# rmqtt/rmqtt

Measured on NVIDIA H100. Metric: topic-matches/sec @10M subs, higher is better.
Workload: dtype u32

## Files before the change

rmqtt_b200/csrc/engine.cu:

```cuda
#include <cuda_runtime.h>
#include <sched.h>
#include <sys/syscall.h>
#include <unistd.h>

#include <algorithm>
#include <cctype>
#include <cstddef>
#include <cstdio>
#include <cstdlib>
#include <cstring>
#include <condition_variable>
#include <mutex>
#include <string>
#include <type_traits>
#include <vector>

#include "../../include/gpumqtt.h"
#include "host_trie.h"
#include "comm.cuh"
#include "pipeline.cuh"
#include "relations.cuh"
#include "retain_tree.h"
#include "router_host.h"

// ... 320 lines not shown
            if (stage_used_) { CUDA_TRY(cudaEventRecord(ev_arena_[arena_], side)); arena_pending_[arena_] = true; }
            dev_view = trie_view(trie, d_edges.as<EdgeSlot>(), d_ranges.as<Range>(), d_values.as<u32>(), d_dict.as<DictSlot>(), d_pool.as<u8>(), d_cfilter.as<u32>(),
                                 d_tree_slots.as<u32>());
            dev_rview = retain_view(rtree, d_rkids.as<RKid>(), d_redges.as<REdge>(), d_rvals.as<u32>());
            view_epoch++;
            CUDA_TRY(cudaEventRecord(ev_flush, side));
            flush_gen++;
        }
        if (r_shipped) rtree.shipped();
        return GM_OK;
    }

    std::vector<MatchCtx*> all_ctxs() { std::vector<MatchCtx*> v; for (auto& c : ctxs) v.push_back(&c); v.push_back(&devctx); return v; }

    struct MatchCall : MatchIO {
        u64* d_needed = nullptr;
        bool keep_cursor = false;
        bool timing = true;
        u32 site_bits = 0;
    };
    int enqueue_match(MatchCtx& c, MatchCall a, cudaStream_t s) {
        if (a.n == 0) { if (a.d_needed) CUDA_TRY(cudaMemsetAsync(a.d_needed, 0, sizeof(u64), s)); return GM_OK; }
        if (a.n > 0xFFFFFFF0ull) { g_err = "batch too large"; return GM_ERR_TOO_LARGE; }
        if (a.cap > 0xFFFFFFFFull) a.cap = 0xFFFFFFFFull;
        MatchKnobs kn = knobs;
        if (a.site_bits) { kn.site_bits = a.site_bits; kn.sub_bits = 0; }
        const bool small = a.hdr != nullptr;
        const MatchPlan p = plan_match(static_cast<u32>(a.n), dev_view.max_depth, kn, num_sms, small);
        CUDA_TRY(c.d_tok.ensure(p.tok));
        CUDA_TRY(c.d_tok8.ensure(p.tok8));
        CUDA_TRY(c.d_meta.ensure(p.meta));
        CUDA_TRY(c.d_slow.ensure(p.slow));
        CUDA_TRY(c.d_ctrl.ensure(p.ctrl));
        CUDA_TRY(c.d_sort.ensure(p.sort));
        CUDA_TRY(c.d_hist.ensure(p.hist));
        CUDA_TRY(c.d_gstack.ensure(p.gstack));
        CUDA_TRY(c.d_gpool.ensure(p.gpool));
        if (!small) {
            CUDA_TRY(cudaStreamWaitEvent(s, ev_flush, 0));
            if (c.recorded) CUDA_TRY(cudaStreamWaitEvent(s, c.ev_done, 0));
        }
        if (a.keep_cursor) CUDA_TRY(cudaMemsetAsync(static_cast<char*>(c.d_ctrl.p) + sizeof(unsigned long long), 0, sizeof(Ctrl) - sizeof(unsigned long long), s));
        else CUDA_TRY(cudaMemsetAsync(c.d_ctrl.p, 0, sizeof(Ctrl), s));
        CUDA_TRY(cudaMemsetAsync(c.d_hist.p, 0, p.nbuckets * sizeof(u32), s));
        MatchScratch m{};
        m.tok = c.d_tok.as<u32>(); m.tok8 = c.d_tok8.as<u32>(); m.meta = c.d_meta.as<u32>(); m.slow = c.d_slow.as<u32>(); m.sort = c.d_sort.as<u32>(); m.hist = c.d_hist.as<u32>();
        m.ctrl = c.d_ctrl.as<Ctrl>(); m.gstack = c.d_gstack.as<u64>(); m.gpool = c.d_gpool.as<Desc>();
        cudaEvent_t* ev_t = ev_ring[ring_n % RING];
        cudaError_t ev = cudaSuccess;
        launch_match(p, m, a, kn, dev_view, s, [&](int k) { if (a.timing && ev == cudaSuccess) ev = cudaEventRecord(ev_t[k], s); });
        CUDA_TRY(ev);
        CUDA_TRY(cudaGetLastError());
        if (a.timing) ring_n++;
        launches += 5;
        if (a.d_needed) CUDA_TRY(cudaMemcpyAsync(a.d_needed, &m.ctrl->cursor, sizeof(u64), cudaMemcpyDeviceToDevice, s));
        if (!small) { CUDA_TRY(cudaEventRecord(c.ev_done, s)); c.recorded = true; }
        return GM_OK;
    }

    int enqueue_retain(const void* d_blob_, u64 blob_bytes, const u32* d_offs_, u64 n, gm_span* d_spans_, u32* d_ids_, u64 cap_ids, int32_t* d_status_, cudaStream_t s) {
        std::lock_guard<std::mutex> gd(mu_dev);
        MatchCtx& c = devctx;
        const RetainPlan p = plan_retain(static_cast<u32>(n), dev_rview.max_depth, r_cap_items, r_cap_desc, num_sms);
        CUDA_TRY(c.d_tok.ensure(p.tok));
        CUDA_TRY(c.d_tok8.ensure(p.tok8));
        CUDA_TRY(c.d_meta.ensure(p.meta));
        CUDA_TRY(d_rq.ensure(p.rq));
        CUDA_TRY(d_rctl.ensure(p.ctl));
        CUDA_TRY(d_rfront[0].ensure(p.front));
        CUDA_TRY(d_rfront[1].ensure(p.front));
        CUDA_TRY(d_rdescs.ensure(p.descs));
        CUDA_TRY(cudaStreamWaitEvent(s, ev_flush, 0));
        if (c.recorded) CUDA_TRY(cudaStreamWaitEvent(s, c.ev_done, 0));
        CUDA_TRY(cudaMemsetAsync(d_rctl.p, 0, p.ctl, s));
        CUDA_TRY(cudaMemsetAsync(d_rq.p, 0, p.rq, s));
        RetainScratch r{};
        r.tok = c.d_tok.as<u32>(); r.tok8 = c.d_tok8.as<u32>(); r.meta = c.d_meta.as<u32>(); r.rq = d_rq.as<u32>(); r.ctl = d_rctl.as<RCtl>();
        r.front[0] = d_rfront[0].as<RTask>(); r.front[1] = d_rfront[1].as<RTask>(); r.descs = d_rdescs.as<RDesc>();
        cudaEvent_t* ev_t = ev_ring[ring_n % RING];
        cudaError_t ev = cudaSuccess;
        launch_retain(p, r, dev_view, dev_rview, d_blob_, blob_bytes, d_offs_, d_spans_, d_ids_, cap_ids, d_status_, knobs.retain_stats, s,
                      [&](int k) { if (ev == cudaSuccess) ev = cudaEventRecord(ev_t[k], s); });
        CUDA_TRY(ev);
        CUDA_TRY(cudaGetLastError());
        ring_n++;
        launches += 4 + p.depth + 1;
        CUDA_TRY(cudaEventRecord(c.ev_done, s));
        c.recorded = true;
        return GM_OK;
    }

    int run_retain(const void* d_blob_, u64 blob_bytes, const u32* d_offs_, u64 n, gm_span* d_spans_, u32* d_ids_, u64 cap_ids, int32_t* d_status_, cudaStream_t s, u64* total) {
        for (int attempt = 0; attempt < 12; ++attempt) {
            int st = enqueue_retain(d_blob_, blob_bytes, d_offs_, n, d_spans_, d_ids_, cap_ids, d_status_, s);
            if (st != GM_OK) return st;
            RCtl h{};
            CUDA_TRY(cudaMemcpyAsync(&h, d_rctl.p, sizeof(RCtl), cudaMemcpyDeviceToHost, s));
            CUDA_TRY(cudaStreamSynchronize(s));
            if (h.err == 0 && knobs.retain_stats) {
                const u32 depth = dev_rview.max_depth;
                std::vector<u32> cnt(static_cast<size_t>(depth + 3) * RQ);
                CUDA_TRY(cudaMemcpy(cnt.data(), static_cast<char*>(d_rctl.p) + offsetof(RCtl, counts), cnt.size() * sizeof(u32), cudaMemcpyDeviceToHost));
                fprintf(stderr, "retain stats: visited %llu probes %llu hits %llu; tasks per round:", h.stats[0], h.stats[1], h.grand);
                for (u32 l = 0; l <= depth + 1; ++l) { unsigned long long t = 0; for (u32 k = 0; k < RQ; ++k) t += cnt[static_cast<size_t>(l) * RQ + k]; fprintf(stderr, " %llu", t); }
                unsigned long long nd = 0; for (u32 k = 0; k < RQ; ++k) nd += h.n_desc[k];
                fprintf(stderr, "; descriptors %llu\n", nd);
            }
// ... 267 lines not shown
    }
    const bool desc = elem == 8;
    auto enqueue = [&](cudaStream_t s) -> int {
        char* di = static_cast<char*>(g->d_in.p);
        char* dout = static_cast<char*>(g->d_out.p);
        gm_engine::MatchCall a;
        a.blob = di + g->off_blob; a.blob_bytes = a.readable_bytes = g->cap_blob; a.offs = reinterpret_cast<const u32*>(di + g->off_offs); a.n = g->cap_n;
        a.hdr = reinterpret_cast<const u32*>(di); a.trees = reinterpret_cast<const u32*>(di + g->off_trees);
        a.spans = reinterpret_cast<gm_span*>(dout + g->off_spans); a.out = dout + g->off_out; a.cap = g->cap_out; a.d_needed = reinterpret_cast<u64*>(dout);
        a.status = reinterpret_cast<int32_t*>(dout + g->off_status); a.desc = desc; a.timing = false; a.site_bits = 10u;
        return e->enqueue_match(c, a, s);
    };
    if (!g->warmed) {
        CUDA_TRY(cudaMemsetAsync(g->d_in.p, 0, g->in_bytes, c.sc));
        int st = enqueue(c.sc);
        if (st != GM_OK) return st;
        CUDA_TRY(cudaStreamSynchronize(c.sc));
        g->warmed = true;
    }
    if (g->exec && g->scratch_sig != c.scratch_sig()) {
        CUDA_TRY(cudaMemsetAsync(g->d_in.p, 0, g->in_bytes, c.sc));
        int st = enqueue(c.sc);
        if (st != GM_OK) return st;
        CUDA_TRY(cudaStreamSynchronize(c.sc));
    }
    if (!g->exec || g->view_epoch != e->view_epoch || g->elem != elem || g->scratch_sig != c.scratch_sig()) {
        cudaGraph_t graph = nullptr;
        CUDA_TRY(cudaStreamBeginCapture(c.sc, cudaStreamCaptureModeRelaxed));
        cudaError_t ce = cudaMemcpyAsync(g->d_in.p, g->h_in, g->in_bytes, cudaMemcpyHostToDevice, c.sc);
        int st = ce == cudaSuccess ? enqueue(c.sc) : GM_ERR_CUDA;
        if (st == GM_OK) ce = cudaMemcpyAsync(g->h_out, g->d_out.p, g->out_bytes, cudaMemcpyDeviceToHost, c.sc);
        cudaError_t ee = cudaStreamEndCapture(c.sc, &graph);
        if (st != GM_OK || ce != cudaSuccess || ee != cudaSuccess) { if (graph) cudaGraphDestroy(graph); g_err = "small-batch graph capture failed"; return st != GM_OK ? st : GM_ERR_CUDA; }
        bool ok = false;
        if (g->exec) {
            cudaGraphExecUpdateResultInfo info{};
            ok = cudaGraphExecUpdate(g->exec, graph, &info) == cudaSuccess;
            if (!ok) { cudaGetLastError(); cudaGraphExecDestroy(g->exec); g->exec = nullptr; }
        }
        if (!ok) CUDA_TRY(cudaGraphInstantiate(&g->exec, graph, 0));
        cudaGraphDestroy(graph);
        g->view_epoch = e->view_epoch; g->elem = elem; g->scratch_sig = c.scratch_sig();
    }
    u32* hdr = reinterpret_cast<u32*>(g->h_in);
    hdr[0] = static_cast<u32>(n); hdr[1] = static_cast<u32>(blob_bytes);
    u32* ho = reinterpret_cast<u32*>(g->h_in + g->off_offs);
    for (u64 i = 0; i <= n; ++i) ho[i] = static_cast<u32>(offsets[i] - b0);
    if (blob_bytes) std::memcpy(g->h_in + g->off_blob, blob + b0, blob_bytes);
    if (trees) std::memcpy(g->h_in + g->off_trees, trees, n * sizeof(u32)); else std::memset(g->h_in + g->off_trees, 0, n * sizeof(u32));
    CUDA_TRY(cudaStreamWaitEvent(c.sc, e->ev_flush, 0));
    CUDA_TRY(cudaGraphLaunch(g->exec, c.sc));
    CUDA_TRY(cudaEventRecord(c.ev_done, c.sc));
    c.recorded = true;
    e->launches += 5;
    gd.unlock();
    CUDA_TRY(cudaEventSynchronize(c.ev_done));
    const u64 total = *reinterpret_cast<const u64*>(g->h_out);
    if (total > g->cap_out) return GM_SMALL_NOT_APPLICABLE;
    if (needed) *needed = total;
    std::memcpy(status, g->h_out + g->off_status, n * sizeof(int32_t));
    if (total > cap_user) { g_err = "output buffer too small"; return GM_ERR_CAPACITY; }
    std::memcpy(out_spans, g->h_out + g->off_spans, n * sizeof(gm_span));
    if (total) std::memcpy(out, g->h_out + g->off_out, total * elem);
    return GM_OK;
}

extern "C" {

struct CtxLease {
    gm_engine* e; MatchCtx* c = nullptr;
    explicit CtxLease(gm_engine* e_) : e(e_) {}
    void acquire(std::unique_lock<std::mutex>& lk) {
        for (;;) {
            for (auto& cx : e->ctxs) if (!cx.busy) { cx.busy = true; c = &cx; return; }
            e->cv_ctx.wait(lk);
        }
    }
    ~CtxLease() {
        if (!c) return;
        { std::lock_guard<std::mutex> g(e->mu_dev); c->busy = false; }
        e->cv_ctx.notify_one();
    }
};

static int32_t match_host_impl(gm_engine* e, const char* blob, const uint32_t* offsets, uint64_t n, gm_span* out_spans, void* out, size_t elem,
                               uint64_t cap_ids, uint64_t* needed, int32_t* status, const uint32_t* trees = nullptr) {
    if (!e || (n && (!offsets || !out_spans || !status)) || (cap_ids && !out)) return GM_ERR_INVALID_ARG;
    if (needed) *needed = 0;
    if (n == 0) return GM_OK;
    if (n > 0xFFFFFFF0ull) { g_err = "batch too large"; return GM_ERR_TOO_LARGE; }
    const bool desc = elem == 8;
    if (e->flags & GM_FLAG_HOST_ONLY) { g_err = "host-only engine cannot match: there is no CPU fallback"; return GM_ERR_NO_DEVICE; }
    CUDA_TRY(cudaSetDevice(e->device));
    { int st = auto_flush(e); if (st != GM_OK) return st; }
    const u64 blob_bytes = offsets[n];
    if (cap_ids > 0xFFFFFFFFull) cap_ids = 0xFFFFFFFFull;
    CtxLease lease(e);
    std::unique_lock<std::mutex> gd(e->mu_dev);
    lease.acquire(gd);
    MatchCtx& c = *lease.c;
    if (e->knobs.small_graphs) {
        int st = small_graph_match(e, c, gd, blob, offsets, n, out_spans, out, elem, cap_ids, needed, status, trees);
        if (st != GM_SMALL_NOT_APPLICABLE) return st;
        if (!gd.owns_lock()) gd.lock();
    }
    CUDA_TRY(c.d_blob.ensure(blob_bytes + 16));
    CUDA_TRY(c.d_offs.ensure((n + 1) * sizeof(u32)));
// ... 816 lines not shown
```

rmqtt_b200/csrc/kernels.cuh:

```cuda
#pragma once
#include <cuda_runtime.h>

#include "layout.h"

#ifdef GM_CPU_EMU
#define GM_LAUNCH(k, grid, block, smem, s, ...) emu::launch(dim3(grid), dim3(block), [&] { k(__VA_ARGS__); })
#else
#define GM_LAUNCH(k, grid, block, smem, s, ...) k<<<grid, block, smem, s>>>(__VA_ARGS__)
#endif

namespace gm {

struct MatchParams {
    TrieView tv;
    const u32* tok8;
    const u32* tok;
    const u32* meta;
    u32 n;
    u32 tok_levels;
    uint2* spans;
    u32* out_ids;
    unsigned long long cap_ids;
    unsigned long long* cursor;
    u32* slow_list;
    u32* slow_count;
    u32* tile_counter;
    unsigned long long* stats;
    u32 flags;
    const u32* perm;
    const u32* tok8_sorted;
    const u32* meta_sorted;
    u32 tile_chunk;
    u32* g_ids[8];
    uint2* g_spans[8];
    u32* g_index[8];
    u32 g_world;
    u32 g_base_topics;
    unsigned long long g_base_ids;
    const u32* g_sel;
    const u32* trees;
    const u32* n_ptr;
    uint2* out_desc;
    int* status;
};
constexpr u32 MP_DIAG_NO_PUBLISH = 2u;
constexpr u32 MP_SORTED_ROWS = 1u;
constexpr u32 MAX_BUCKET_BITS = 18;
constexpr u32 TOK8 = 8;
constexpr u32 K2_SMEM_DESCS = 8;
template <int FAST_L, int THREADS> constexpr size_t k2_smem_bytes() { return (2 * sizeof(u32) * FAST_L + sizeof(uint2) * K2_SMEM_DESCS) * THREADS; }

#ifndef GM_CPU_EMU
__device__ __forceinline__ void ld256(const void* p, u32 (&w)[8]) {
    asm volatile("ld.global.nc.v4.u32 {%0,%1,%2,%3}, [%8];\n\t"
                 "ld.global.nc.v4.u32 {%4,%5,%6,%7}, [%8+16];"
                 : "=r"(w[0]), "=r"(w[1]), "=r"(w[2]), "=r"(w[3]), "=r"(w[4]), "=r"(w[5]), "=r"(w[6]), "=r"(w[7])
                 : "l"(p));
}
__device__ __forceinline__ void st256(void* p, const u32 (&w)[8]) {
    asm volatile("st.global.v4.u32 [%0], {%1,%2,%3,%4};\n\t"
                 "st.global.v4.u32 [%0+16], {%5,%6,%7,%8};" ::"l"(p), "r"(w[0]), "r"(w[1]), "r"(w[2]), "r"(w[3]), "r"(w[4]), "r"(w[5]), "r"(w[6]), "r"(w[7]) : "memory");
}
__device__ __forceinline__ u32 lanemask_lt() {
    u32 m;
    asm("mov.u32 %0, %%lanemask_lt;" : "=r"(m));
    return m;
}
#else
inline void ld256(const void* p, u32 (&w)[8]) { __builtin_memcpy(w, p, 32); }
inline void st256(void* p, const u32 (&w)[8]) { __builtin_memcpy(p, w, 32); }
inline u32 lanemask_lt() { return (1u << (threadIdx.x & 31u)) - 1u; }
#endif

constexpr int TOK_THREADS = 256;

__device__ __forceinline__ u32 swar_zero_bytes(u32 v) { return (v - 0x01010101u) & ~v & 0x80808080u; }

__device__ __forceinline__ u32 text4(const u8* a, const u8* limit) {
    const uintptr_t ai = reinterpret_cast<uintptr_t>(a);
    const u32* w = reinterpret_cast<const u32*>(ai & ~uintptr_t(3));
    const u32 lo = reinterpret_cast<const u8*>(w) < limit ? __ldg(w) : 0u;
    const u32 hi = reinterpret_cast<const u8*>(w + 1) < limit ? __ldg(w + 1) : 0u;
    return __funnelshift_r(lo, hi, 8u * static_cast<u32>(ai & 3));
}

__device__ __forceinline__ u32 text4_s(const u32* stage, u32 off) {
    const u32 lo = stage[off >> 2], hi = stage[(off >> 2) + 1];
    return __funnelshift_r(lo, hi, 8u * (off & 3u));
}

#ifndef GM_CPU_EMU
__device__ __forceinline__ u32 smem_u32(const void* p) { return static_cast<u32>(__cvta_generic_to_shared(p)); }
__device__ __forceinline__ void mbar_init(unsigned long long* bar, u32 count) {
    asm volatile("mbarrier.init.shared::cta.b64 [%0], %1;" ::"r"(smem_u32(bar)), "r"(count) : "memory");
}
__device__ __forceinline__ void mbar_expect_tx(unsigned long long* bar, u32 bytes) {
    asm volatile("mbarrier.arrive.expect_tx.shared::cta.b64 _, [%0], %1;" ::"r"(smem_u32(bar)), "r"(bytes) : "memory");
// ... 199 lines not shown
}

constexpr u32 KIND_PROBE = 0, KIND_PLUS = 1;
__device__ __forceinline__ u64 make_item(u32 topic, u32 depth, u32 kind, u32 arg, u32 wtag = 0u) {
    return (static_cast<u64>(topic | (depth << 5) | (kind << 21) | (wtag << 22)) << 32) | arg;
}

struct NodeRec { u32 node, plus, hash_ref, own_ref, mask, cnts; };

__device__ __forceinline__ bool load_record(const TrieView& tv, u32 kind, u32 arg, u32 token, u32 pmask_tag, NodeRec& r) {
    u32 s[8];
    if (kind == KIND_PLUS) {
        ld256(tv.edges + (arg - 1u), s);
        r.node = s[2]; r.plus = s[3]; r.hash_ref = s[4]; r.own_ref = s[5]; r.mask = s[6]; r.cnts = s[7];
        return true;
    }
    u32 idx = edge_slot0(arg, token, pmask_tag >> WTAG_SHIFT, tv.win_mask, tv.win_shift, tv.nwin_mask);
    for (;;) {
        ld256(tv.edges + idx, s);
        if (s[2] == 0) return false;
        if (s[0] == arg && s[1] == token) break;
        idx = edge_next(idx, tv.win_mask);
    }
    r.node = s[2]; r.plus = s[3]; r.hash_ref = s[4]; r.own_ref = s[5]; r.mask = s[6]; r.cnts = s[7];
    return true;
}

__device__ __forceinline__ bool cfilter_maybe(const TrieView& tv, u32 parent, u32 token) {
    u32 w, bits;
    cfilter_pos(parent, token, tv.cfilter_mask, w, bits);
    return (__ldg(tv.cfilter + w) & bits) == bits;
}

__device__ __forceinline__ u32 next_tile_chunked(unsigned long long* s_chunk, u32* s_lock, u32* gcounter, u32 chunk) {
    for (;;) {
        unsigned long long cur = *reinterpret_cast<volatile unsigned long long*>(s_chunk);
        if (static_cast<u32>(cur) < static_cast<u32>(cur >> 32)) {
            if (atomicCAS(s_chunk, cur, cur + 1ull) == cur) return static_cast<u32>(cur);
            continue;
        }
        if (atomicCAS(s_lock, 0u, 1u) == 0u) {
            cur = *reinterpret_cast<volatile unsigned long long*>(s_chunk);
            if (static_cast<u32>(cur) < static_cast<u32>(cur >> 32)) { atomicExch(s_lock, 0u); continue; }
            const u32 base = atomicAdd(gcounter, chunk);
            atomicExch(s_chunk, (static_cast<unsigned long long>(base + chunk) << 32) | (base + 1u));
            __threadfence_block();
            atomicExch(s_lock, 0u);
            return base;
        }
    }
}

struct Desc { u32 ref, cnt; };

template <int FAST_L, int THREADS, int CTAS_PER_SM, bool STATS, bool DESC, bool GATHER = false>
__global__ void __launch_bounds__(THREADS, CTAS_PER_SM)
k_match_fast(MatchParams p, Desc* __restrict__ dpool, u32 pool_rows) {
    static_assert(!(GATHER && DESC), "the fused gather publishes ids");
    constexpr u32 SD = K2_SMEM_DESCS;
#ifndef GM_CPU_EMU
    extern __shared__ __align__(16) unsigned char k2_smem[];
#else
    unsigned char* k2_smem = emu::dyn_smem();
#endif
    u32 (*s_tok)[THREADS] = reinterpret_cast<u32 (*)[THREADS]>(k2_smem);
    u32 (*s_pend)[THREADS] = reinterpret_cast<u32 (*)[THREADS]>(k2_smem + sizeof(u32) * FAST_L * THREADS);
    uint2 (*s_desc)[THREADS] = reinterpret_cast<uint2 (*)[THREADS]>(k2_smem + 2 * sizeof(u32) * FAST_L * THREADS);
    const u32 tid = threadIdx.x, lane = tid & 31;
    const u32 lt = lanemask_lt();
    const u32 nthreads = gridDim.x * THREADS;
    const u32 gtid = blockIdx.x * THREADS + tid;
    const TrieView& tv = p.tv;
    const u32 n_act = p.n_ptr ? min(p.n, *p.n_ptr) : p.n;
    const u32 ntiles = (n_act + 31) >> 5;
    unsigned long long sV = 0, sE = 0, sF = 0, sM = 0;
    __shared__ unsigned long long s_chunk;
    __shared__ u32 s_lock;
    const u32 chunk = p.tile_chunk;
    if (chunk > 1) {
        if (tid == 0) { s_chunk = 0ull; s_lock = 0u; }
        __syncthreads();
    }
    for (;;) {
        u32 tile = 0;
        if (lane == 0) tile = chunk > 1 ? next_tile_chunked(&s_chunk, &s_lock, p.tile_counter, chunk) : atomicAdd(p.tile_counter, 1u);
        tile = __shfl_sync(0xFFFFFFFFu, tile, 0);
        if (tile >= ntiles) break;

        const u32 pos = tile * 32 + lane;
        const bool in_range = pos < n_act;
        const u32 t = in_range ? p.perm[pos] : 0u;
        const bool rows = (p.flags & MP_SORTED_ROWS) != 0;
        const u32 m = in_range ? (rows ? __ldcs(p.meta_sorted + pos) : __ldcs(p.meta + t)) : META_INVALID;
        const bool invalid = (m & META_INVALID) != 0;
        const u32 L = m & META_NLEV_MASK;
        const u32 need = min(L, tv.max_depth);
        const bool slow_pre = in_range && !invalid && need > FAST_L;
        const bool active = in_range && !invalid && !slow_pre;
        bool defer = slow_pre;
        u32 ndesc = 0, total = 0;

        if (active) {
            {
                static_assert(FAST_L == TOK8, "the token row holds 8 levels");
                u32 w[8];
                ld256(rows ? p.tok8_sorted + static_cast<size_t>(pos) * TOK8 : p.tok8 + static_cast<size_t>(t) * TOK8, w);
// ... 41 lines not shown
                            probe = true; kp = r.node; kt = tk; nd = d + 1;
                            idx = edge_slot0(kp, kt, r.mask >> WTAG_SHIFT, tv.win_mask, tv.win_shift, tv.nwin_mask);
                            if (STATS) atomicAdd(p.stats + 4 + min(d, 7u), 1ull);
                        }
                    }
                }
                droot = false;
                bool done = false;
                u32 s[8];
                for (;;) {
                    if (!probe) {
                        if (pmask == 0) { done = true; break; }
                        const u32 pd = 31u - __clz(pmask);
                        pmask &= ~(1u << pd);
                        idx = s_pend[pd][tid] - 1u;
                        nd = pd + 1;
                    }
                    ld256(tv.edges + idx, s);
                    if (!probe) break;
                    if (STATS) atomicAdd(p.stats + 20, 1ull);
                    if (s[2] == 0) {
                        if (STATS) atomicAdd(p.stats + 12 + min(nd - 1u, 7u), 1ull);
                        probe = false;
                        continue;
                    }
                    if (s[0] == kp && s[1] == kt) break;
                    idx = edge_next(idx, tv.win_mask);
                }
                if (done) break;
                r.node = s[2]; r.plus = s[3]; r.hash_ref = s[4]; r.own_ref = s[5]; r.mask = s[6]; r.cnts = s[7];
                d = nd;
            }
            if (STATS && !defer) { sV += lV; sE += lE; sF += lF; sM += total; }
        }

        const u32 nd = (active && !defer) ? ndesc : 0u;
        const u32 mine = DESC ? nd : ((active && !defer) ? total : 0u);
        u32 inc = mine;
#pragma unroll
        for (int o = 1; o < 32; o <<= 1) { u32 v = __shfl_up_sync(0xFFFFFFFFu, inc, o); if (lane >= o) inc += v; }
        const u32 wtotal = __shfl_sync(0xFFFFFFFFu, inc, 31);
        const u32 pre = inc - mine;
        unsigned long long base = 0;
        if (lane == 0 && wtotal) base = atomicAdd(p.cursor, static_cast<unsigned long long>(wtotal));
        base = __shfl_sync(0xFFFFFFFFu, base, 0);
        const bool fits = base + wtotal <= p.cap_ids;
        if (in_range && !defer) {
            if (GATHER) {
                const uint2 gsp = make_uint2(fits ? static_cast<u32>(p.g_base_ids + base + pre) : 0u, mine);
                const u32 gi = p.g_sel ? p.g_sel[t] : t;
                for (u32 w = 0; w < p.g_world; ++w) { p.g_spans[w][p.g_base_topics + t] = gsp; p.g_index[w][p.g_base_topics + t] = gi; }
            } else p.spans[t] = make_uint2(fits ? static_cast<u32>(base + pre) : 0u, mine);
        }
        const u32 maxd = __reduce_max_sync(0xFFFFFFFFu, nd);
        if (DESC) {
            if (fits && wtotal) {
                uint2* __restrict__ outd = p.out_desc + base + pre;
                for (u32 k = 0; k < nd; ++k) {
                    uint2 v;
                    if (k < SD) v = s_desc[k][tid];
                    else { const Desc dd = dpool[static_cast<size_t>(k - SD) * nthreads + gtid]; v = make_uint2(dd.ref, dd.cnt); }
                    __stcs(outd + k, v);
                }
            }
        } else if (fits && wtotal && !(p.flags & MP_DIAG_NO_PUBLISH)) {
            u32* __restrict__ out = p.out_ids + base;
            u32 cur = pre;
            for (u32 k = 0; k < maxd; ++k) {
                Desc dsc{0u, 0u};
                if (k < nd) {
                    if (k < SD) { const uint2 v = s_desc[k][tid]; dsc = Desc{v.x, v.y}; }
                    else dsc = dpool[static_cast<size_t>(k - SD) * nthreads + gtid];
                }
                const u32 ni = dsc.cnt;
                const u32 dst = cur;
                cur += ni;
                u32 sc = ni;
#pragma unroll
                for (int o = 1; o < 32; o <<= 1) { u32 v = __shfl_up_sync(0xFFFFFFFFu, sc, o); if (lane >= o) sc += v; }
                const u32 tot = __shfl_sync(0xFFFFFFFFu, sc, 31);
                const u32 exc = sc - ni;
                const u32 delta = dst - exc, gamma = dsc.ref - exc;
                const u32 single = __ballot_sync(0xFFFFFFFFu, ni == 1u);
                for (u32 e0 = 0; e0 < tot; e0 += 32) {
                    const u32 e = e0 + lane;
                    u32 lo = 0;
#pragma unroll
                    for (int step = 16; step; step >>= 1) {
                        u32 v = __shfl_sync(0xFFFFFFFFu, exc, lo + step);
                        if (v <= e) lo += step;
                    }
                    const u32 o_delta = __shfl_sync(0xFFFFFFFFu, delta, lo);
                    const u32 o_gamma = __shfl_sync(0xFFFFFFFFu, gamma, lo);
                    if (e < tot) {
                        const u32 src = e + o_gamma;
                        const u32 val = ((single >> lo) & 1u) ? src : tv.values[src];
                        if (GATHER) {
                            const unsigned long long at = p.g_base_ids + base + e + o_delta;
                            for (u32 w = 0; w < p.g_world; ++w) p.g_ids[w][at] = val;
                        } else __stcs(out + e + o_delta, val);
                    }
                }
            }
        }
        const bool deferred = in_range && defer;
        u32 db = __ballot_sync(0xFFFFFFFFu, deferred);
        if (db) {
            u32 sb = 0;
            if (lane == 0) sb = atomicAdd(p.slow_count, static_cast<u32>(__popc(db)));
            sb = __shfl_sync(0xFFFFFFFFu, sb, 0);
            if (deferred) p.slow_list[sb + __popc(db & lt)] = t;
        }
    }
    if (STATS) {
#pragma unroll
        for (int o = 16; o; o >>= 1) {
            sV += __shfl_xor_sync(0xFFFFFFFFu, sV, o); sE += __shfl_xor_sync(0xFFFFFFFFu, sE, o);
            sF += __shfl_xor_sync(0xFFFFFFFFu, sF, o); sM += __shfl_xor_sync(0xFFFFFFFFu, sM, o);
        }
        if (lane == 0) { atomicAdd(p.stats + 0, sV); atomicAdd(p.stats + 1, sE); atomicAdd(p.stats + 2, sF); atomicAdd(p.stats + 3, sM); }
    }
}

template <bool STATS, bool DESC, bool GATHER = false>
__global__ void __launch_bounds__(256)
k_match_slow(MatchParams p, u64* __restrict__ gstack, u32 stack_cap) {
    auto put = [&](unsigned long long at, u32 v) {
        if (GATHER) { for (u32 w = 0; w < p.g_world; ++w) p.g_ids[w][p.g_base_ids + at] = v; }
        else p.out_ids[at] = v;
    };
    const u32 lane = threadIdx.x & 31;
    const u32 lt = lanemask_lt();
    const u32 gwarp = (blockIdx.x * blockDim.x + threadIdx.x) >> 5;
    const u32 nwarps = (gridDim.x * blockDim.x) >> 5;
    const TrieView& tv = p.tv;
    u64* stack = gstack + static_cast<size_t>(gwarp) * stack_cap;
    const u32 nslow = *p.slow_count;
    unsigned long long sV = 0, sE = 0, sF = 0, sM = 0;

    for (u32 si = gwarp; si < nslow; si += nwarps) {
        const u32 t = p.slow_list[si];
        const u32 m = p.meta[t];
        const u32 L = m & META_NLEV_MASK;
        const bool dollar = (m & META_DOLLAR) != 0;
        unsigned long long base = 0;
        unsigned long long count = 0;
        bool fits = true, bad_any = false;
        for (int pass = 0; pass < 2; ++pass) {
            u32 stack_n = 0;
            unsigned long long written = 0;
            bool bad = false;
            auto consume = [&](bool hit, u32 d, const NodeRec& r, bool dollar_root) {
                const u32 c1 = (hit && !dollar_root) ? (r.cnts & 0xFFFFu) : 0u;
                const u32 c2 = (hit && d == L) ? (r.cnts >> 16) : 0u;
                u64 itA = 0, itB = 0;
                bool pA = false, pB = false;
                if (hit && d < L) {
                    const u32 plus_idx = r.plus;
                    if (plus_idx != 0 && !dollar_root) { pA = true; itA = make_item(0, d + 1, KIND_PLUS, plus_idx); }
                    if ((r.mask & MASK_BLOOM) != 0 && d < p.tok_levels) {
                        u32 tk = d < TOK8 ? p.tok8[static_cast<size_t>(t) * TOK8 + d] : p.tok[static_cast<size_t>(d) * p.n + t];
                        if (tk != TOK_UNKNOWN && (r.mask & mask_bit(tk)) && (!(r.mask & MASK_WIDE_FLAG) || cfilter_maybe(tv, r.node, tk))) {
                            pB = true; itB = make_item(0, d + 1, KIND_PROBE, r.node, r.mask >> WTAG_SHIFT);
                        }
                    }
                }
                if (STATS && pass == 0) { sV += hit; sE += (hit && d < L); }
#pragma unroll
                for (int round = 0; round < 2; ++round) {
                    const u32 cn = round == 0 ? c1 : c2;
                    const u32 ref = round == 0 ? r.hash_ref : r.own_ref;
                    if (STATS && pass == 0) sF += (cn != 0);
                    if (DESC) {
// ... 103 lines not shown
```

rmqtt_b200/csrc/pipeline.cuh:

```cuda
#pragma once
#include <algorithm>
#include <cstddef>

#include "../../include/gpumqtt.h"
#include "host_trie.h"
#include "kernels.cuh"
#include "retain_kernels.cuh"
#include "retain_tree.h"

namespace gm {

struct Ctrl { unsigned long long cursor; unsigned long long stats[24]; u32 slow_count; u32 tile_counter; };

struct RCtl {
    unsigned long long grand; unsigned long long stats[2]; u32 err; u32 pad; u32 n_desc[RQ]; u32 counts[RQ];
    static size_t bytes(u32 depth) { return sizeof(RCtl) + static_cast<size_t>(depth + 3) * RQ * sizeof(u32) + static_cast<size_t>(depth + 3) * sizeof(u32); }
    u32* round_counts(u32 lvl) { return counts + static_cast<size_t>(lvl) * RQ; }
    u32* claim(u32 depth, u32 lvl) { return counts + static_cast<size_t>(depth + 3) * RQ + lvl; }
};

constexpr int K2_FAST_L = 8;
constexpr int K2_THREADS = 512;
constexpr int K2_CTAS_PER_SM = 3;
constexpr u32 K2_POOL_ROWS = 24;
constexpr size_t K2_SMEM = k2_smem_bytes<K2_FAST_L, K2_THREADS>();

inline auto k2_kernel(bool stats, bool desc, bool gather) {
    return gather ? k_match_fast<K2_FAST_L, K2_THREADS, K2_CTAS_PER_SM, false, false, true>
         : stats  ? (desc ? k_match_fast<K2_FAST_L, K2_THREADS, K2_CTAS_PER_SM, true, true> : k_match_fast<K2_FAST_L, K2_THREADS, K2_CTAS_PER_SM, true, false>)
                  : (desc ? k_match_fast<K2_FAST_L, K2_THREADS, K2_CTAS_PER_SM, false, true> : k_match_fast<K2_FAST_L, K2_THREADS, K2_CTAS_PER_SM, false, false>);
}
inline auto k3_kernel(bool stats, bool desc, bool gather) {
    return gather ? k_match_slow<false, false, true>
         : stats  ? (desc ? k_match_slow<true, true> : k_match_slow<true, false>) : (desc ? k_match_slow<false, true> : k_match_slow<false, false>);
}

struct MatchKnobs { u32 site_bits = 14, sub_bits = 0; bool sorted_rows = true; int k2_ctas = 0; u32 diag_flags = 0; u32 tile_chunk = 1; bool tok_bulk = true; u32 pool_rows = K2_POOL_ROWS; };

inline size_t tok_bytes(u32 tok_levels, u32 n) { return tok_levels > TOK8 ? static_cast<size_t>(tok_levels) * n * sizeof(u32) : 256; }

struct MatchPlan {
    u32 n, tok_levels, nbuckets, stack_cap, pool_rows;
    int tok_grid, scatter_grid, k2_grid, k3_blocks;
    size_t tok, tok8, meta, slow, ctrl, sort, hist, gstack, gpool;
};
inline MatchPlan plan_match(u32 n, u32 max_depth, const MatchKnobs& kn, int num_sms, bool small) {
    MatchPlan p{};
    p.n = n;
    p.tok_levels = std::max<u32>(1u, max_depth);
    p.nbuckets = 1u << (kn.site_bits + kn.sub_bits);
    p.stack_cap = 32u * (max_depth + 2u) + 64u;
    p.pool_rows = kn.pool_rows;
    const int k2_ctas = (kn.k2_ctas >= 1 && kn.k2_ctas <= K2_CTAS_PER_SM) ? kn.k2_ctas : K2_CTAS_PER_SM;
    p.tok_grid = static_cast<int>((n + TOK_THREADS - 1) / TOK_THREADS);
    p.scatter_grid = static_cast<int>((n + 255) / 256);
    p.k2_grid = small ? std::max(1, std::min<int>(num_sms * k2_ctas, (n + K2_THREADS - 1) / K2_THREADS)) : num_sms * k2_ctas;
    p.k3_blocks = small ? std::max(1, std::min<int>(num_sms, (n + 7) / 8)) : num_sms * 4;
    p.tok = tok_bytes(p.tok_levels, n); p.tok8 = static_cast<size_t>(n) * TOK8 * sizeof(u32);
    p.meta = p.slow = n * sizeof(u32); p.ctrl = sizeof(Ctrl);
    p.sort = static_cast<size_t>(n) * 11 * sizeof(u32) + 64;
    p.hist = 2 * static_cast<size_t>(p.nbuckets) * sizeof(u32);
    p.gstack = static_cast<size_t>(num_sms) * 4 * 8 * p.stack_cap * sizeof(u64);
    p.gpool = static_cast<size_t>(num_sms) * k2_ctas * K2_THREADS * p.pool_rows * sizeof(Desc);
    return p;
}

struct RetainPlan {
    u32 nq, depth, tok_levels, slice_items, slice_desc;
    int tok_grid, init_grid, round_grid, expand_grid;
    size_t tok, tok8, meta, rq, ctl, front, descs;
};
inline RetainPlan plan_retain(u32 nq, u32 depth, u32 cap_items, u32 cap_desc, int num_sms) {
    RetainPlan p{};
    p.nq = nq; p.depth = depth;
    p.tok_levels = depth + 2;
    p.slice_items = std::max<u32>(1u, cap_items / RQ); p.slice_desc = std::max<u32>(1u, cap_desc / RQ);
    p.tok_grid = static_cast<int>((nq + TOK_THREADS - 1) / TOK_THREADS);
    p.init_grid = static_cast<int>((nq + 255) / 256);
    p.round_grid = num_sms * GM_RETAIN_CTAS;
    p.expand_grid = num_sms * 8;
    p.tok = tok_bytes(p.tok_levels, nq); p.tok8 = static_cast<size_t>(nq) * TOK8 * sizeof(u32); p.meta = nq * sizeof(u32);
    p.rq = static_cast<size_t>(nq) * 3 * sizeof(u32); p.ctl = RCtl::bytes(depth);
    p.front = static_cast<size_t>(p.slice_items) * RQ * sizeof(RTask); p.descs = static_cast<size_t>(p.slice_desc) * RQ * sizeof(RDesc);
    return p;
}

struct GatherLayout {
    static constexpr size_t off_ids = 256;
    u32 world = 0; u64 slab_topics = 0, slab_ids = 0;
    size_t off_spans = 0, off_index = 0, off_counts = 0, off_flags = 0, bytes = 0;
};
inline GatherLayout gather_layout(u32 world, u64 slab_topics, u64 slab_ids) {
    GatherLayout g;
    g.world = world; g.slab_topics = (slab_topics + 3) & ~u64(3); g.slab_ids = (slab_ids + 3) & ~u64(3);
    const size_t a = 256;
    g.off_spans = (GatherLayout::off_ids + static_cast<size_t>(world) * g.slab_ids * 4 + a - 1) / a * a;
    g.off_index = g.off_spans + static_cast<size_t>(world) * g.slab_topics * 8;
    g.off_counts = (g.off_index + static_cast<size_t>(world) * g.slab_topics * 4 + a - 1) / a * a;
    g.off_flags = g.off_counts + static_cast<size_t>(world) * 16;
    g.bytes = g.off_flags + 256;
    return g;
}
struct GatherTarget { const GatherLayout* layout; char* const* blocks; u32 rank; bool direct; };

struct MatchScratch { u32 *tok, *tok8, *meta, *slow, *sort, *hist; Ctrl* ctrl; u64* gstack; Desc* gpool; };

struct MatchIO {
    const void* blob = nullptr; u64 blob_bytes = 0, readable_bytes = 0;
    const u32* offs = nullptr;
    const u32* sel = nullptr;
    u64 n = 0;
    const u32* hdr = nullptr;
    const u32* trees = nullptr;
    gm_span* spans = nullptr; void* out = nullptr; u64 cap = 0;
    int32_t* status = nullptr;
    bool stats = false, desc = false;
    const GatherTarget* gather = nullptr;
};

struct NoHook { void operator()(int) const {} };

template <class Hook = NoHook>
inline void launch_match(const MatchPlan& p, const MatchScratch& m, const MatchIO& io, const MatchKnobs& kn, const TrieView& tv, cudaStream_t s, Hook at = {}) {
    const u32 n = p.n;
    u32* bkey = m.sort;
    u32* perm = bkey + n;
    u32* meta_sorted = perm + n;
    u32* tok8_sorted = meta_sorted + n + ((8 - (3 * static_cast<size_t>(n)) % 8) % 8);
    u32* bcursor = m.hist + p.nbuckets;
    at(0);
    auto k1 = kn.tok_bulk ? k_tokenize<true> : k_tokenize<false>;
    GM_LAUNCH(k1, p.tok_grid, TOK_THREADS, 0, s, static_cast<const u8*>(io.blob), static_cast<u32>(io.blob_bytes), static_cast<u32>(std::max<u64>(io.blob_bytes, io.readable_bytes)),
              io.offs, io.sel, n, io.hdr, tv, p.tok_levels, m.tok8, m.tok, m.meta, io.status, bkey, m.hist, kn.site_bits, kn.sub_bits);
    GM_LAUNCH(k_bucket_scan, 1, 1024, 0, s, m.hist, bcursor, p.nbuckets);
    GM_LAUNCH(k_bucket_scatter, p.scatter_grid, 256, 0, s, bkey, bcursor, n, io.hdr, perm, m.tok8, m.meta, kn.sorted_rows ? tok8_sorted : nullptr, meta_sorted);
    at(1);
    MatchParams mp{};
    mp.tv = tv; mp.tok8 = m.tok8; mp.tok = m.tok; mp.meta = m.meta; mp.n = n; mp.n_ptr = io.hdr; mp.tok_levels = p.tok_levels;
    mp.spans = reinterpret_cast<uint2*>(io.spans); mp.out_ids = static_cast<u32*>(io.out); mp.out_desc = static_cast<uint2*>(io.out); mp.cap_ids = io.cap;
    mp.status = io.status;
    mp.trees = io.trees;
    mp.cursor = &m.ctrl->cursor; mp.slow_list = m.slow; mp.slow_count = &m.ctrl->slow_count;
    mp.tile_counter = &m.ctrl->tile_counter; mp.stats = m.ctrl->stats;
    mp.perm = perm; mp.tok8_sorted = tok8_sorted; mp.meta_sorted = meta_sorted;
    mp.flags = (kn.sorted_rows ? MP_SORTED_ROWS : 0u) | kn.diag_flags;
    mp.tile_chunk = kn.tile_chunk;
    if (const GatherTarget* g = io.gather) {
        const GatherLayout& L = *g->layout;
        mp.g_base_topics = static_cast<u32>(g->rank * L.slab_topics); mp.g_base_ids = g->rank * L.slab_ids; mp.g_sel = io.sel;
        mp.g_world = g->direct ? L.world : 1;
        for (u32 w = 0; w < mp.g_world; ++w) {
            char* b = g->blocks[g->direct ? w : g->rank];
            mp.g_ids[w] = reinterpret_cast<u32*>(b + GatherLayout::off_ids); mp.g_spans[w] = reinterpret_cast<uint2*>(b + L.off_spans);
            mp.g_index[w] = reinterpret_cast<u32*>(b + L.off_index);
        }
    }
    const bool gather = io.gather != nullptr;
    auto k2 = k2_kernel(io.stats, io.desc, gather);
    GM_LAUNCH(k2, p.k2_grid, K2_THREADS, K2_SMEM, s, mp, m.gpool, p.pool_rows);
    at(2);
    auto k3 = k3_kernel(io.stats, io.desc, gather);
    GM_LAUNCH(k3, p.k3_blocks, 256, 0, s, mp, m.gstack, p.stack_cap);
    at(3);
}

struct RetainScratch { u32 *tok, *tok8, *meta, *rq; RCtl* ctl; RTask* front[2]; RDesc* descs; };

template <class Hook = NoHook>
inline void launch_retain(const RetainPlan& p, const RetainScratch& r, const TrieView& tv, const RetainView& rv, const void* blob, u64 blob_bytes, const u32* offs,
                          gm_span* spans, u32* ids, u64 cap_ids, int32_t* status, bool stats, cudaStream_t s, Hook at = {}) {
    const u32 nq = p.nq, depth = p.depth;
    u32* qtotal = r.rq;
    u32* qbase = qtotal + nq;
    u32* qcur = qbase + nq;
    at(0);
    GM_LAUNCH(k_tokenize<false>, p.tok_grid, TOK_THREADS, 0, s, static_cast<const u8*>(blob), static_cast<u32>(blob_bytes), static_cast<u32>(blob_bytes), offs, nullptr, nq, nullptr, tv,
              p.tok_levels, r.tok8, r.tok, r.meta, status, nullptr, nullptr, 0u, 0u);
    at(1);
    RetainParams rp{};
    rp.v = rv; rp.qtok8 = r.tok8; rp.qtok = r.tok; rp.qmeta = r.meta; rp.nq = nq; rp.tok_levels = p.tok_levels;
    rp.descs = r.descs; rp.n_desc = r.ctl->n_desc; rp.cap_items = p.slice_items; rp.cap_desc = p.slice_desc;
    rp.qtotal = qtotal; rp.err = &r.ctl->err;
    rp.stats = r.ctl->stats;
    auto kri = stats ? k_retain_init<true> : k_retain_init<false>;
    auto krr = stats ? k_retain_round<true> : k_retain_round<false>;
    GM_LAUNCH(kri, p.init_grid, 256, 0, s, rp, r.front[0], r.ctl->round_counts(0));
    for (u32 lvl = 0; lvl <= depth; ++lvl)
        GM_LAUNCH(krr, p.round_grid, 256, 0, s, rp, r.front[lvl & 1], r.ctl->round_counts(lvl), r.front[(lvl + 1) & 1], r.ctl->round_counts(lvl + 1), r.ctl->claim(depth, lvl));
    at(2);
    GM_LAUNCH(k_retain_scan, 1, 1024, 0, s, qtotal, nq, qbase, reinterpret_cast<uint2*>(spans), &r.ctl->grand);
    GM_LAUNCH(k_retain_expand, p.expand_grid, 256, 0, s, r.descs, r.ctl->n_desc, p.slice_desc, rv.vals, qbase, qcur, ids, cap_ids);
    at(3);
}

inline void launch_tokenize(bool bulk, const void* blob, u64 blob_bytes, const u32* offs, u32 n, const TrieView& tv, u32 tok_levels, u32* tok8, u32* tok, u32* meta,
                            int32_t* status, cudaStream_t s) {
    auto k = bulk ? k_tokenize<true> : k_tokenize<false>;
    GM_LAUNCH(k, (n + TOK_THREADS - 1) / TOK_THREADS, TOK_THREADS, 0, s, static_cast<const u8*>(blob), static_cast<u32>(blob_bytes), static_cast<u32>((blob_bytes + 15) & ~u64(15)),
              offs, nullptr, n, nullptr, tv, tok_levels, tok8, tok, meta, status, nullptr, nullptr, 0u, 0u);
}

inline TrieView trie_view(const HostTrie& t, const EdgeSlot* edges, const Range* ranges, const u32* values, const DictSlot* dict, const u8* pool, const u32* cfilter,
                          const u32* tree_slots) {
    TrieView v{};
    v.edges = edges; v.ranges = ranges; v.values = values; v.dict = dict; v.pool = pool;
    v.cfilter = cfilter; v.cfilter_mask = static_cast<u32>(t.cfilter.size() - 1);
    v.edge_mask = static_cast<u32>(t.edges.size() - 1);
    v.win_mask = t.win_mask(); v.win_shift = t.win_shift(); v.nwin_mask = t.nwin_mask();
    v.dict_mask = static_cast<u32>(t.dict.size() - 1);
    v.root_plus = t.root_plus; v.root_hash_ref = t.root_hash_ref; v.root_hash_cnt = t.root_hash_cnt; v.root_mask = t.root_mask;
    v.max_depth = t.max_depth;
    v.tree_slots = tree_slots; v.n_trees = tree_slots ? static_cast<u32>(t.tree_slots.size()) : 0u;
// ... 24 lines not shown
```

rmqtt_b200/csrc/retain_kernels.cuh:

```cuda
#pragma once
#include <cuda_runtime.h>

#include "kernels.cuh"
#include "retain_tree.h"

namespace gm {

struct alignas(16) RDesc { u32 q, ref, cnt, kind; };

struct alignas(16) RTask { u32 q, pos_mode, kb, kn; };
constexpr u32 RTASK_CHUNK = 256;

constexpr u32 RQ = 64;

struct RetainParams {
    RetainView v;
    const u32* qtok8;
    const u32* qtok;
    const u32* qmeta;
    u32 nq, tok_levels;
    RDesc* descs;
    u32* n_desc;
    u32 cap_items, cap_desc;
    u32* qtotal;
// ... 223 lines not shown
    }
    if (STATS) {
#pragma unroll
        for (int o = 16; o; o >>= 1) { visited += __shfl_xor_sync(0xFFFFFFFFu, visited, o); probes += __shfl_xor_sync(0xFFFFFFFFu, probes, o); }
        if (lane == 0 && (visited | probes)) { atomicAdd(p.stats, visited); atomicAdd(p.stats + 1, probes); }
    }
}

__global__ void __launch_bounds__(1024)
k_retain_scan(const u32* __restrict__ qtotal, u32 nq, u32* __restrict__ qbase, uint2* __restrict__ spans, unsigned long long* grand) {
    __shared__ unsigned long long s_part[1024];
    const u32 tid = threadIdx.x;
    const u32 per = (nq + 1023) / 1024;
    const u32 b = min(nq, tid * per), e = min(nq, b + per);
    unsigned long long sum = 0;
    for (u32 i = b; i < e; ++i) sum += qtotal[i];
    s_part[tid] = sum;
    __syncthreads();
    if (tid == 0) {
        unsigned long long run = 0;
        for (int i = 0; i < 1024; ++i) { unsigned long long x = s_part[i]; s_part[i] = run; run += x; }
        *grand = run;
    }
    __syncthreads();
    unsigned long long run = s_part[tid];
    for (u32 i = b; i < e; ++i) {
        const u32 c = qtotal[i];
        const u32 off = run > 0xFFFFFFFFull ? 0xFFFFFFFFu : static_cast<u32>(run);
        qbase[i] = off;
        spans[i] = make_uint2(off, c);
        run += c;
    }
}

__global__ void __launch_bounds__(256)
k_retain_expand(const RDesc* __restrict__ descs, const u32* __restrict__ n_desc_p, u32 cap_desc, const u32* __restrict__ rvals,
                const u32* __restrict__ qbase, u32* __restrict__ qcur, u32* __restrict__ out, unsigned long long cap_ids) {
    const u32 lane = threadIdx.x & 31;
    const u32 gwarp = (blockIdx.x * blockDim.x + threadIdx.x) >> 5, nwarps = (gridDim.x * blockDim.x) >> 5;
    __shared__ u32 s_pre[RQ + 1];
    const u32 nd = queue_prefix(n_desc_p, cap_desc, s_pre);
    for (u32 base = gwarp * 32; base < nd; base += nwarps * 32) {
        const u32 i = base + lane;
        RDesc d = i < nd ? descs[queue_locate(s_pre, i, cap_desc)] : RDesc{0, 0, 0, 0};
        const u32 ni = d.cnt;
        const u32 dst = ni ? qbase[d.q] + atomicAdd(qcur + d.q, ni) : 0u;
        u32 sc = ni;
#pragma unroll
        for (int o = 1; o < 32; o <<= 1) { u32 x = __shfl_up_sync(0xFFFFFFFFu, sc, o); if (lane >= o) sc += x; }
        const u32 tot = __shfl_sync(0xFFFFFFFFu, sc, 31);
        const u32 exc = sc - ni;
        for (u32 e0 = 0; e0 < tot; e0 += 32) {
            const u32 e = e0 + lane;
            u32 lo = 0;
#pragma unroll
            for (int step = 16; step; step >>= 1) {
                u32 x = __shfl_sync(0xFFFFFFFFu, exc, lo + step);
                if (x <= e) lo += step;
            }
            const u32 o_exc = __shfl_sync(0xFFFFFFFFu, exc, lo);
            const u32 o_ref = __shfl_sync(0xFFFFFFFFu, d.ref, lo);
            const u32 o_kind = __shfl_sync(0xFFFFFFFFu, d.kind, lo);
            const u32 o_dst = __shfl_sync(0xFFFFFFFFu, dst, lo);
            if (e < tot) {
                const u32 k = e - o_exc;
                const unsigned long long at = static_cast<unsigned long long>(o_dst) + k;
                if (at < cap_ids) __stcs(out + at, o_kind ? rvals[o_ref + k] : o_ref);
            }
        }
    }
}

}
```

Before: 1.058 billion.

## Split match ID expansion into a separate per-tile expand kernel

The k2 match kernel no longer expands descriptors into subscriber IDs inline. Each warp now writes its descriptors to a compacted item buffer through a global atomic cursor and records a per-tile record; a new k_match_expand kernel then expands items into output IDs, one warp per tile. The aim is to take the divergent, latency-heavy expansion loop out of the register- and smem-heavy k2 kernel so that it runs with a better load balance. In exchange it adds a kernel launch, a global round trip for descriptors, and a large extra scratch allocation (32 descriptors per topic).

```diff
diff --git a/rmqtt_b200/csrc/engine.cu b/rmqtt_b200/csrc/engine.cu
--- a/rmqtt_b200/csrc/engine.cu
+++ b/rmqtt_b200/csrc/engine.cu
@@ -396,7 +396,7 @@
         CUDA_TRY(ev);
         CUDA_TRY(cudaGetLastError());
         if (a.timing) ring_n++;
-        launches += 5;
+        launches += a.desc ? 5 : 6;
         if (a.d_needed) CUDA_TRY(cudaMemcpyAsync(a.d_needed, &m.ctrl->cursor, sizeof(u64), cudaMemcpyDeviceToDevice, s));
         if (!small) { CUDA_TRY(cudaEventRecord(c.ev_done, s)); c.recorded = true; }
         return GM_OK;
@@ -770,7 +770,7 @@
     CUDA_TRY(cudaGraphLaunch(g->exec, c.sc));
     CUDA_TRY(cudaEventRecord(c.ev_done, c.sc));
     c.recorded = true;
-    e->launches += 5;
+    e->launches += desc ? 5 : 6;
     gd.unlock();
     CUDA_TRY(cudaEventSynchronize(c.ev_done));
     const u64 total = *reinterpret_cast<const u64*>(g->h_out);
diff --git a/rmqtt_b200/csrc/kernels.cuh b/rmqtt_b200/csrc/kernels.cuh
--- a/rmqtt_b200/csrc/kernels.cuh
+++ b/rmqtt_b200/csrc/kernels.cuh
@@ -42,7 +42,12 @@
     const u32* n_ptr;
     uint2* out_desc;
     int* status;
+    uint2* items;
+    struct TileRec* tiles;
+    unsigned long long* item_cursor;
 };
+struct TileRec { u32 item_base, n_items; unsigned long long id_base; };
+static_assert(sizeof(TileRec) == 16, "one 16-byte record per tile");
 constexpr u32 MP_DIAG_NO_PUBLISH = 2u;
 constexpr u32 MP_SORTED_ROWS = 1u;
 constexpr u32 MAX_BUCKET_BITS = 18;
@@ -348,6 +353,16 @@
 }
 
 struct Desc { u32 ref, cnt; };
+
+__device__ __forceinline__ u32 warp_run_owner(u32 exc, u32 e) {
+    u32 lo = 0;
+#pragma unroll
+    for (int step = 16; step; step >>= 1) {
+        const u32 v = __shfl_sync(0xFFFFFFFFu, exc, lo + step);
+        if (v <= e) lo += step;
+    }
+    return lo;
+}
 
 template <int FAST_L, int THREADS, int CTAS_PER_SM, bool STATS, bool DESC, bool GATHER = false>
 __global__ void __launch_bounds__(THREADS, CTAS_PER_SM)
@@ -495,56 +510,27 @@
                 for (u32 w = 0; w < p.g_world; ++w) { p.g_spans[w][p.g_base_topics + t] = gsp; p.g_index[w][p.g_base_topics + t] = gi; }
             } else p.spans[t] = make_uint2(fits ? static_cast<u32>(base + pre) : 0u, mine);
         }
-        const u32 maxd = __reduce_max_sync(0xFFFFFFFFu, nd);
+        auto store_descs = [&](uint2* __restrict__ outd) {
+            for (u32 k = 0; k < nd; ++k) {
+                uint2 v;
+                if (k < SD) v = s_desc[k][tid];
+                else { const Desc dd = dpool[static_cast<size_t>(k - SD) * nthreads + gtid]; v = make_uint2(dd.ref, dd.cnt); }
+                __stcs(outd + k, v);
+            }
+        };
         if (DESC) {
-            if (fits && wtotal) {
-                uint2* __restrict__ outd = p.out_desc + base + pre;
-                for (u32 k = 0; k < nd; ++k) {
-                    uint2 v;
-                    if (k < SD) v = s_desc[k][tid];
-                    else { const Desc dd = dpool[static_cast<size_t>(k - SD) * nthreads + gtid]; v = make_uint2(dd.ref, dd.cnt); }
-                    __stcs(outd + k, v);
-                }
-            }
-        } else if (fits && wtotal && !(p.flags & MP_DIAG_NO_PUBLISH)) {
-            u32* __restrict__ out = p.out_ids + base;
-            u32 cur = pre;
-            for (u32 k = 0; k < maxd; ++k) {
-                Desc dsc{0u, 0u};
-                if (k < nd) {
-                    if (k < SD) { const uint2 v = s_desc[k][tid]; dsc = Desc{v.x, v.y}; }
-                    else dsc = dpool[static_cast<size_t>(k - SD) * nthreads + gtid];
-                }
-                const u32 ni = dsc.cnt;
-                const u32 dst = cur;
-                cur += ni;
-                u32 sc = ni;
-#pragma unroll
-                for (int o = 1; o < 32; o <<= 1) { u32 v = __shfl_up_sync(0xFFFFFFFFu, sc, o); if (lane >= o) sc += v; }
-                const u32 tot = __shfl_sync(0xFFFFFFFFu, sc, 31);
-                const u32 exc = sc - ni;
-                const u32 delta = dst - exc, gamma = dsc.ref - exc;
-                const u32 single = __ballot_sync(0xFFFFFFFFu, ni == 1u);
-                for (u32 e0 = 0; e0 < tot; e0 += 32) {
-                    const u32 e = e0 + lane;
-                    u32 lo = 0;
-#pragma unroll
-                    for (int step = 16; step; step >>= 1) {
-                        u32 v = __shfl_sync(0xFFFFFFFFu, exc, lo + step);
-                        if (v <= e) lo += step;
-                    }
-                    const u32 o_delta = __shfl_sync(0xFFFFFFFFu, delta, lo);
-                    const u32 o_gamma = __shfl_sync(0xFFFFFFFFu, gamma, lo);
-                    if (e < tot) {
-                        const u32 src = e + o_gamma;
-                        const u32 val = ((single >> lo) & 1u) ? src : tv.values[src];
-                        if (GATHER) {
-                            const unsigned long long at = p.g_base_ids + base + e + o_delta;
-                            for (u32 w = 0; w < p.g_world; ++w) p.g_ids[w][at] = val;
-                        } else __stcs(out + e + o_delta, val);
-                    }
-                }
-            }
+            if (fits && wtotal) store_descs(p.out_desc + base + pre);
+        } else {
+            const u32 ni = (fits && !(p.flags & MP_DIAG_NO_PUBLISH)) ? nd : 0u;
+            u32 iinc = ni;
+#pragma unroll
+            for (int o = 1; o < 32; o <<= 1) { u32 v = __shfl_up_sync(0xFFFFFFFFu, iinc, o); if (lane >= o) iinc += v; }
+            const u32 witems = __shfl_sync(0xFFFFFFFFu, iinc, 31);
+            u32 ibase = 0;
+            if (lane == 0 && witems) ibase = static_cast<u32>(atomicAdd(p.item_cursor, static_cast<unsigned long long>(witems)));
+            ibase = __shfl_sync(0xFFFFFFFFu, ibase, 0);
+            if (lane == 0) p.tiles[tile] = TileRec{ibase, witems, base};
+            if (ni) store_descs(p.items + ibase + (iinc - ni));
         }
         const bool deferred = in_range && defer;
         u32 db = __ballot_sync(0xFFFFFFFFu, deferred);
@@ -562,6 +548,41 @@
             sF += __shfl_xor_sync(0xFFFFFFFFu, sF, o); sM += __shfl_xor_sync(0xFFFFFFFFu, sM, o);
         }
         if (lane == 0) { atomicAdd(p.stats + 0, sV); atomicAdd(p.stats + 1, sE); atomicAdd(p.stats + 2, sF); atomicAdd(p.stats + 3, sM); }
+    }
+}
+
+template <bool GATHER>
+__global__ void __launch_bounds__(256)
+k_match_expand(MatchParams p) {
+    const u32 lane = threadIdx.x & 31;
+    const u32 gwarp = (blockIdx.x * blockDim.x + threadIdx.x) >> 5, nwarps = (gridDim.x * blockDim.x) >> 5;
+    const u32 n_act = p.n_ptr ? min(p.n, *p.n_ptr) : p.n;
+    const u32 ntiles = (n_act + 31) >> 5;
+    for (u32 tile = gwarp; tile < ntiles; tile += nwarps) {
+        const TileRec rec = p.tiles[tile];
+        unsigned long long at = (GATHER ? p.g_base_ids : 0ull) + rec.id_base;
+        for (u32 i0 = 0; i0 < rec.n_items; i0 += 32) {
+            const u32 i = i0 + lane;
+            const uint2 d = i < rec.n_items ? __ldcs(p.items + rec.item_base + i) : make_uint2(0u, 0u);
+            u32 sc = d.y;
+#pragma unroll
+            for (int o = 1; o < 32; o <<= 1) { u32 v = __shfl_up_sync(0xFFFFFFFFu, sc, o); if (lane >= o) sc += v; }
+            const u32 tot = __shfl_sync(0xFFFFFFFFu, sc, 31);
+            const u32 exc = sc - d.y;
+            const u32 gamma = d.x - exc;
+            const u32 single = __ballot_sync(0xFFFFFFFFu, d.y == 1u);
+            for (u32 e0 = 0; e0 < tot; e0 += 32) {
+                const u32 e = e0 + lane;
+                const u32 o = warp_run_owner(exc, e);
+                const u32 src = e + __shfl_sync(0xFFFFFFFFu, gamma, o);
+                if (e < tot) {
+                    const u32 val = ((single >> o) & 1u) ? src : p.tv.values[src];
+                    if (GATHER) { for (u32 w = 0; w < p.g_world; ++w) p.g_ids[w][at + e] = val; }
+                    else __stcs(p.out_ids + at + e, val);
+                }
+            }
+            at += tot;
+        }
     }
 }
 
diff --git a/rmqtt_b200/csrc/pipeline.cuh b/rmqtt_b200/csrc/pipeline.cuh
--- a/rmqtt_b200/csrc/pipeline.cuh
+++ b/rmqtt_b200/csrc/pipeline.cuh
@@ -10,7 +10,7 @@
 
 namespace gm {
 
-struct Ctrl { unsigned long long cursor; unsigned long long stats[24]; u32 slow_count; u32 tile_counter; };
+struct Ctrl { unsigned long long cursor; unsigned long long item_cursor; unsigned long long stats[24]; u32 slow_count; u32 tile_counter; };
 
 struct RCtl {
     unsigned long long grand; unsigned long long stats[2]; u32 err; u32 pad; u32 n_desc[RQ]; u32 counts[RQ];
@@ -41,7 +41,7 @@
 
 struct MatchPlan {
     u32 n, tok_levels, nbuckets, stack_cap, pool_rows;
-    int tok_grid, scatter_grid, k2_grid, k3_blocks;
+    int tok_grid, scatter_grid, k2_grid, expand_grid, k3_blocks;
     size_t tok, tok8, meta, slow, ctrl, sort, hist, gstack, gpool;
 };
 inline MatchPlan plan_match(u32 n, u32 max_depth, const MatchKnobs& kn, int num_sms, bool small) {
@@ -55,10 +55,11 @@
     p.tok_grid = static_cast<int>((n + TOK_THREADS - 1) / TOK_THREADS);
     p.scatter_grid = static_cast<int>((n + 255) / 256);
     p.k2_grid = small ? std::max(1, std::min<int>(num_sms * k2_ctas, (n + K2_THREADS - 1) / K2_THREADS)) : num_sms * k2_ctas;
+    p.expand_grid = small ? std::max(1, std::min<int>(num_sms * 8, (n + 255) / 256)) : num_sms * 8;
     p.k3_blocks = small ? std::max(1, std::min<int>(num_sms, (n + 7) / 8)) : num_sms * 4;
     p.tok = tok_bytes(p.tok_levels, n); p.tok8 = static_cast<size_t>(n) * TOK8 * sizeof(u32);
     p.meta = p.slow = n * sizeof(u32); p.ctrl = sizeof(Ctrl);
-    p.sort = static_cast<size_t>(n) * 11 * sizeof(u32) + 64;
+    p.sort = static_cast<size_t>(n) * 11 * sizeof(u32) + 64 + static_cast<size_t>((n + 31) / 32) * sizeof(TileRec) + 32ull * n * sizeof(uint2);
     p.hist = 2 * static_cast<size_t>(p.nbuckets) * sizeof(u32);
     p.gstack = static_cast<size_t>(num_sms) * 4 * 8 * p.stack_cap * sizeof(u64);
     p.gpool = static_cast<size_t>(num_sms) * k2_ctas * K2_THREADS * p.pool_rows * sizeof(Desc);
@@ -127,6 +128,8 @@
     u32* perm = bkey + n;
     u32* meta_sorted = perm + n;
     u32* tok8_sorted = meta_sorted + n + ((8 - (3 * static_cast<size_t>(n)) % 8) % 8);
+    TileRec* tiles = reinterpret_cast<TileRec*>(tok8_sorted + static_cast<size_t>(n) * TOK8);
+    uint2* items = reinterpret_cast<uint2*>(tiles + (n + 31) / 32);
     u32* bcursor = m.hist + p.nbuckets;
     at(0);
     auto k1 = kn.tok_bulk ? k_tokenize<true> : k_tokenize<false>;
@@ -139,6 +142,7 @@
     mp.tv = tv; mp.tok8 = m.tok8; mp.tok = m.tok; mp.meta = m.meta; mp.n = n; mp.n_ptr = io.hdr; mp.tok_levels = p.tok_levels;
     mp.spans = reinterpret_cast<uint2*>(io.spans); mp.out_ids = static_cast<u32*>(io.out); mp.out_desc = static_cast<uint2*>(io.out); mp.cap_ids = io.cap;
     mp.status = io.status;
+    mp.items = items; mp.tiles = tiles; mp.item_cursor = &m.ctrl->item_cursor;
     mp.trees = io.trees;
     mp.cursor = &m.ctrl->cursor; mp.slow_list = m.slow; mp.slow_count = &m.ctrl->slow_count;
     mp.tile_counter = &m.ctrl->tile_counter; mp.stats = m.ctrl->stats;
@@ -158,6 +162,10 @@
     const bool gather = io.gather != nullptr;
     auto k2 = k2_kernel(io.stats, io.desc, gather);
     GM_LAUNCH(k2, p.k2_grid, K2_THREADS, K2_SMEM, s, mp, m.gpool, p.pool_rows);
+    if (!io.desc) {
+        auto kx = gather ? k_match_expand<true> : k_match_expand<false>;
+        GM_LAUNCH(kx, p.expand_grid, 256, 0, s, mp);
+    }
     at(2);
     auto k3 = k3_kernel(io.stats, io.desc, gather);
     GM_LAUNCH(k3, p.k3_blocks, 256, 0, s, mp, m.gstack, p.stack_cap);
diff --git a/rmqtt_b200/csrc/retain_kernels.cuh b/rmqtt_b200/csrc/retain_kernels.cuh
--- a/rmqtt_b200/csrc/retain_kernels.cuh
+++ b/rmqtt_b200/csrc/retain_kernels.cuh
@@ -299,12 +299,7 @@
         const u32 exc = sc - ni;
         for (u32 e0 = 0; e0 < tot; e0 += 32) {
             const u32 e = e0 + lane;
-            u32 lo = 0;
-#pragma unroll
-            for (int step = 16; step; step >>= 1) {
-                u32 x = __shfl_sync(0xFFFFFFFFu, exc, lo + step);
-                if (x <= e) lo += step;
-            }
+            const u32 lo = warp_run_owner(exc, e);
             const u32 o_exc = __shfl_sync(0xFFFFFFFFu, exc, lo);
             const u32 o_ref = __shfl_sync(0xFFFFFFFFu, d.ref, lo);
             const u32 o_kind = __shfl_sync(0xFFFFFFFFu, d.kind, lo);
```

After: 1.245 billion, median of 6. 1.18x the previous value.
